# airl-iisc/MRFP

Measured on AMD Instinct MI355X. Metric: train images/sec, higher is better.
Workload: dtype bf16; 1 GPU; resnet-101 DeepLabV3+ + MRFP+ (HRFP+NP+ on, HRFP re-drawn every step), 768x768, 16 images/GPU, fwd+bwd+SGD, synthetic 19-class, random-init weights; global_batch=16, parallelism=dp1

## Files before the change

include/mrfp_hip.h:

```cpp
#ifndef MRFP_HIP_H
#define MRFP_HIP_H

#include <stdint.h>

#ifdef __cplusplus
extern "C" {
#endif

typedef enum { MRFP_F32 = 0, MRFP_BF16 = 1, MRFP_F16 = 2 } mrfp_dtype;

int mrfp_version(void);
const char* mrfp_last_error(void);

int64_t mrfp_stats_nslab(int64_t B, int64_t Ho);

int mrfp_stats_fwd(const void* x, int dtype, int64_t B, int64_t Ho, int64_t Wo, int64_t C,
                   int64_t Hs, int64_t Ws, const int32_t* tabH, const int32_t* tabW,
                   float* ws, void* stream);

int mrfp_stats_bwd(const void* dy, const void* x, const void* y, const float* mean,
                   const float* fA, const float* fS, int per_image, int dtype, int64_t B, int64_t Ho, int64_t Wo, int64_t C,
                   int64_t Hs, int64_t Ws, const int32_t* tabH, const int32_t* tabW,
                   float* ws, void* stream);
int mrfp_stats_bwd_mask(const void* dy, const void* x, const void* mask, const float* mean, int per_image, int dtype, int64_t B,
// ... 22 lines not shown
int mrfp_np_bwd_finalize(const float* ws, int64_t B, int64_t nslab, int64_t count, int64_t C,
                         const float* alpha, const float* beta_noise, const float* mu,
                         const float* sigma, float* Gtmp , float* K, void* stream);

int mrfp_mean_finalize(const float* ws, int64_t B, int64_t nslab, int64_t count, int64_t C,
                       float* tmp, void* out, int dtype, void* stream);

int mrfp_affine_fwd(const void* x, const void* res, void* y, int dtype,
                    int64_t B, int64_t Ho, int64_t Wo, int64_t C, int64_t Hs, int64_t Ws,
                    const int32_t* tabH, const int32_t* tabW,
                    const float* A, const float* S, int coef_per_image, int relu, void* stream);

int mrfp_affine_fwd_stats(const void* x, const void* res, void* y, int dtype, int64_t B, int64_t H, int64_t W, int64_t C,
                          const float* A, const float* S, int coef_per_image, int relu, float* ws, void* stream);
int mrfp_affine_bwd(const void* dy, const void* x, const void* y, void* dx, void* dres, int dtype,
                    int64_t B, int64_t Ho, int64_t Wo, int64_t C, int64_t Hs, int64_t Ws,
                    const int32_t* invH, const int32_t* invW,
                    const float* P, const float* Q, const float* R,
                    const float* fA, const float* fS, int coef_per_image, void* stream);
int mrfp_affine_fwd_relu_mask(const void* x, const void* res, void* y, void* mask, int dtype, int64_t B, int64_t H, int64_t W,
                              int64_t C, const float* A, const float* S, int coef_per_image, void* stream);
int mrfp_affine_bwd_mask(const void* dy, const void* x, const void* mask, void* dx, void* dres, int dtype, int64_t B, int64_t H,
                         int64_t W, int64_t C, const float* P, const float* Q, const float* R, int coef_per_image, void* stream);

int mrfp_copy_channels(const void* src, void* dst, int dtype, int64_t npix, int64_t C, int64_t ld_src, int64_t c0_src,
                       int64_t ld_dst, int64_t c0_dst, void* stream);

int mrfp_add(const void* a, const void* b, void* y, int dtype, int64_t n, void* stream);

int mrfp_bilinear_fwd(const void* x, const void* addend, void* y, int dtype,
                      int64_t B, int64_t Hi, int64_t Wi, int64_t Ho, int64_t Wo, int64_t C, int64_t ld_in,
                      void* stream);
int mrfp_bilinear_bwd(const void* dy, void* dx, int dtype,
                      int64_t B, int64_t Hi, int64_t Wi, int64_t Ho, int64_t Wo, int64_t C, int64_t ld_in,
                      void* stream);
int mrfp_bilinear_fwd_into(const void* x, void* y, int dtype, int64_t B, int64_t Hi, int64_t Wi, int64_t Ho, int64_t Wo,
                           int64_t C, int64_t ld_in, int64_t ld_out, void* stream);
int mrfp_bilinear_bwd_from(const void* dy, void* dx, int dtype, int64_t B, int64_t Hi, int64_t Wi, int64_t Ho, int64_t Wo,
                           int64_t C, int64_t ld_in, int64_t ld_dy, void* stream);

int mrfp_maxpool_fwd(const void* x, void* y, uint8_t* idx, int dtype,
                     int64_t B, int64_t H, int64_t W, int64_t C, void* stream);
int mrfp_maxpool_bwd(const void* dy, const uint8_t* idx, void* dx, int dtype,
                     int64_t B, int64_t H, int64_t W, int64_t C, void* stream);

int mrfp_maxpool_affine_fwd(const void* x, const float* A, const float* S, int coef_per_image, int relu, void* y, uint8_t* idx,
// ... 199 lines not shown
```

mrfp_amd/conv.py:

```python
from __future__ import annotations

import collections
import ctypes
import os as _os
import warnings
import weakref
from typing import Any, NamedTuple, Optional

import torch

from . import _lib
from ._lib import call, dt, ptr, stream
from .ops import CL, GRAD_DEFERRED, _chk, channel_sums, empty_cl, grad_sink, notify_grad, wgrad_workspace, zeros_cl
from .ops import _inside_autograd_engine as _in_backward

_PACKS = {}
FUSE_STATS = [_os.environ.get("MRFP_FUSE_STATS", "1") != "0"]


class ConvStats(NamedTuple):
    final: torch.Tensor
    final_count: int
    elements: int
    rows: torch.Tensor
# ... 653 lines not shown
            side = _WGRADS.stream(x.device) if sink is not None else None
            if sink is not None and GROUP_WGRAD[0] and L_single(B, H, W, Cphys, Ho, Wo, Nphys, x.element_size()):
                _WGRADS.submit(sig, x, dy, sink, weight)
            elif side is not None:
                _WGRADS.ensure_callback()
                _launch_wgrads(sig, [(x, dy, sink)], side)
                notify_grad(weight)
            else:
                dw = sink if sink is not None else torch.empty((N, C, R, S), dtype=torch.float32, device=x.device)
                _launch_wgrads(sig, [(x, dy, dw)], None)
                if sink is not None:
                    notify_grad(weight)
                    dw = None
                elif dw.dtype != weight.dtype:
                    dw = dw.to(weight.dtype)
        if bias is not None and ctx.needs_input_grad[2]:
            db = channel_sums(dy, N).to(bias.dtype)
        return (dx, dw, db) + (None,) * 8


class _SharedConv1x1Pair(torch.autograd.Function):

    @staticmethod
    def forward(ctx, x1, x2, weight, bias, Nphys):
        N, C, R, S = weight.shape
        if R != 1 or S != 1 or x1.shape[1] != C or x2.shape[1] != C:
            raise _lib.MrfpHipError("shared conv pair: 1x1 weight and unpadded inputs expected")
        pk = get_pack(weight, bias, x1.dtype, C, Nphys)
        ys = []
        for x, b in ((x1, None), (x2, pk.bias)):
            B, _, H, W = x.shape
            y = empty_cl(B, Nphys, H, W, x.dtype, x.device)
            call("mrfp_conv_fwd", ptr(x), ptr(pk.wf), ptr(b), ptr(y), dt(x), B, H, W, C, Nphys, Nphys, 1, 1, H, W, 1, 0, 0, 1, 1,
                 None, None, stream())
            ys.append(y)
        ctx.save_for_backward(x1, x2, weight, bias)
        ctx.Nphys = Nphys
        ctx.lr_cell = getattr(x2, "_mrfp_uses", None) if getattr(x2, "_mrfp_lowrank_ok", False) else None
        ctx.set_materialize_grads(False)
        return ys[0], ys[1]

    @staticmethod
    def backward(ctx, dy1, dy2):
        x1, x2, weight, bias = ctx.saved_tensors
        N, C, _, _ = weight.shape
        Nphys = ctx.Nphys
        pk = get_pack(weight, bias, x1.dtype, C, Nphys)
        dxs, dws = [], []
        db = None
        for x, dy, need_dx, cell in ((x1, dy1, ctx.needs_input_grad[0], None), (x2, dy2, ctx.needs_input_grad[1], ctx.lr_cell)):
            if dy is None:
                dxs.append(None)
                continue
            dy = _chk(dy, "dy")
# ... 4 lines not shown
                dx = torch.empty((), dtype=x.dtype, device=x.device).expand(B, C, H, W)
                dx._mrfp_lowrank = (dy, pk.wd, Nphys, dx._version)
                cell[2] = True
            elif need_dx:
                dx = empty_cl(B, C, H, W, x.dtype, x.device)
                call("mrfp_conv_fwd", ptr(dy), ptr(pk.wd), None, ptr(dx), dt(dy), B, H, W, Nphys, C, C, 1, 1, H, W, 1, 0, 0, 1, 1,
                     None, None, stream())
            dxs.append(dx)
            if ctx.needs_input_grad[2]:
                dw = torch.empty((N, C, 1, 1), dtype=torch.float32, device=x.device)
                _launch_wgrads((x.dtype, B, H, W, C, C, N, Nphys, 1, 1, H, W, 1, 0, 0, 1), [(x, dy, dw)], None)
                dws.append(dw)
        if bias is not None and ctx.needs_input_grad[3] and dy2 is not None:
            db = channel_sums(_chk(dy2, "dy"), N).to(bias.dtype)
        dw = None
        if dws:
            total = dws[0] if len(dws) == 1 else dws[0].add_(dws[1])
            sink = grad_sink(weight)
            if sink is not None:
                sink.copy_(total)
                notify_grad(weight)
            else:
                dw = total.to(weight.dtype)
        return dxs[0], dxs[1], dw, db, None


def shared_conv1x1_pair(x1, x2, weight, bias, phys_out):
    return _SharedConv1x1Pair.apply(_chk(x1), _chk(x2), weight, bias, int(phys_out))


def pad_input_channels(x: torch.Tensor, dtype) -> torch.Tensor:
    if not x.is_cuda:
        raise _lib.MrfpHipError("input must live on the GPU (got %s): the HIP path has no CPU fallback" % x.device)
    B, C, H, W = x.shape
    Cpad = _round_up(C, _epc(dtype))
    xs = x.detach()
    if xs.dtype != torch.float32 or not xs.is_contiguous():
        xs = xs.float().contiguous()
    y = empty_cl(B, Cpad, H, W, dtype, x.device)
    call("mrfp_nchw_to_nhwc_pad", ptr(xs), ptr(y), _lib._DT[dtype], B, C, H, W, Cpad, stream())
    return y


def conv2d(x, weight, bias, stride, padding, dilation, phys_out: Optional[int] = None, want_skip: bool = False,
           groups: int = 1, stat_resize=None):
    st = stride[0] if isinstance(stride, (tuple, list)) else int(stride)
    ph, pw = (padding if isinstance(padding, (tuple, list)) else (int(padding), int(padding)))
    dl = dilation[0] if isinstance(dilation, (tuple, list)) else int(dilation)
    N, C = weight.shape[0], weight.shape[1]
    epc = _epc(x.dtype)
    if x.shape[1] % epc != 0:
# ... 46 lines not shown
```

mrfp_amd/csrc/affine.hip:

```cpp
#include "common.hpp"

namespace mrfp {

template <typename T, int VEC, bool RESIZE>
__global__ __launch_bounds__(kThreads) void affine_fwd_kernel(const T* __restrict__ x, const T* __restrict__ res,
                                                              T* __restrict__ y, RowGeom g, int ly,
                                                              const float* __restrict__ A, const float* __restrict__ S,
                                                              int coef_per_image, int relu, uint8_t* __restrict__ mask_out) {
    const int b = blockIdx.x / ly, j = blockIdx.x % ly;
    const Lanes L = make_lanes(g.C, VEC);
    const int t = threadIdx.x;
    const int tcol = t % L.colthreads, trow = t / L.colthreads;
    if (trow >= L.rowthreads) return;
    const size_t cbase = (size_t)(coef_per_image ? b : 0) * g.C;
    for (int cv = tcol; cv < L.lpr; cv += kThreads) {
        float a[VEC], s[VEC];
#pragma unroll
        for (int i = 0; i < VEC; ++i) { a[i] = 1.f; s[i] = 0.f; }
        if (A) load_coef<VEC>(A + cbase + (size_t)cv * VEC, a);
        if (S) load_coef<VEC>(S + cbase + (size_t)cv * VEC, s);
        for (int oh = j; oh < g.Ho; oh += ly) {
            const int ih = RESIZE ? g.tabH[oh] : oh;
            const T* xl = x ? x + ((size_t)b * g.Hs + ih) * g.Ws * g.C + (size_t)cv * VEC : nullptr;
            const size_t dl = ((size_t)b * g.Ho + oh) * g.Wo * g.C + (size_t)cv * VEC;
// ... 107 lines not shown
                            const float vr = inside ? to_f(from_f<T>(v[i])) : 0.f;
                            su[i] += vr;
                            sq[i] += vr * vr;
                        }
                    }
                }
            }
        }
        __syncthreads();
#pragma unroll
        for (int i = 0; i < VEC; ++i) {
            sm[(t * 2 + 0) * VEC + i] = su[i];
            sm[(t * 2 + 1) * VEC + i] = sq[i];
        }
        __syncthreads();
        const int nout = L.colthreads * 2 * VEC;
        for (int o = t; o < nout; o += kThreads) {
            const int oc = o / (2 * VEC), rest = o % (2 * VEC);
            if (cv0 + oc < L.lpr) {
                float acc = 0.f;
                for (int r = 0; r < L.rowthreads; ++r) acc += sm[((r * L.colthreads + oc) * 2) * VEC + rest];
                const int stat = rest / VEC, i = rest % VEC;
                out[(size_t)stat * g.C + (size_t)(cv0 + oc) * VEC + i] = acc;
            }
        }
    }
}

template <typename T, int VEC, int KR, bool YM = false>
__global__ __launch_bounds__(kThreads) void affine_bwd_kernel(const T* __restrict__ dy, const T* __restrict__ x,
                                                              const T* __restrict__ y, T* __restrict__ dx,
                                                              T* __restrict__ dres, RowGeom g, int ly,
                                                              const int32_t* __restrict__ invH,
                                                              const int32_t* __restrict__ invW,
                                                              const float* __restrict__ P, const float* __restrict__ Q,
                                                              const float* __restrict__ R, const float* __restrict__ fA,
                                                              const float* __restrict__ fS, int coef_per_image) {
    const int b = blockIdx.x / ly, j = blockIdx.x % ly;
    const Lanes L = make_lanes(g.C, VEC);
    const int t = threadIdx.x;
    const int tcol = t % L.colthreads, trow = t / L.colthreads;
    if (trow >= L.rowthreads) return;
    const size_t cbase = (size_t)(coef_per_image ? b : 0) * g.C;
    for (int cv = tcol; cv < L.lpr; cv += kThreads) {
        float p[VEC], q[VEC], r[VEC], fa[VEC], fs[VEC];
#pragma unroll
// ... 217 lines not shown
}

template <typename T>
static int launch_affine_fwd(const void* x, const void* res, void* y, int64_t B, int64_t Ho, int64_t Wo, int64_t C,
                             int64_t Hs, int64_t Ws, const int32_t* tabH, const int32_t* tabW, const float* A,
                             const float* S, int cpi, int relu, hipStream_t st, uint8_t* mask_out = nullptr) {
    RowGeom g{(int)B, (int)Ho, (int)Wo, (int)C, (int)Hs, (int)Ws, tabH, tabW};
    const int ly = lines_per_image(B, Ho);
    dim3 grid((unsigned)(B * ly));
    const bool vec_ok = pick_vec<T>(C) > 1 && (!x || aligned16(x)) && aligned16(y) && (!res || aligned16(res)) &&
                        (!A || aligned16(A)) && (!S || aligned16(S));
    if (mask_out && !(vec_ok && FullVec<T>::value == 8)) { set_error("affine_fwd_mask: 16-bit activations with C %% 8 == 0, 16-byte aligned"); return -1; }
    const bool resize = tabH != nullptr || tabW != nullptr;
    if (resize && !(tabH && tabW)) { set_error("affine_fwd: both index tables or none"); return -1; }
    auto launch = [&](auto rs) {
        constexpr bool RS = decltype(rs)::value != 0;
        MRFP_LAUNCH_VEC(vec_ok, (affine_fwd_kernel<T, FullVec<T>::value, RS>), (affine_fwd_kernel<T, 1, RS>), grid, st, (const T*)x,
                        (const T*)res, (T*)y, g, ly, A, S, cpi, relu, mask_out);
        return 0;
    };
    return resize ? launch(Int<1>{}) : launch(Int<0>{});
}

template <typename T>
static int launch_affine_bwd(const void* dy, const void* x, const void* y, void* dx, void* dres, int64_t B, int64_t Ho,
                             int64_t Wo, int64_t C, int64_t Hs, int64_t Ws, const int32_t* invH, const int32_t* invW,
                             const float* P, const float* Q, const float* R, const float* fA, const float* fS, int cpi,
                             hipStream_t st, bool ymask = false) {
    RowGeom g{(int)B, (int)Ho, (int)Wo, (int)C, (int)Hs, (int)Ws, nullptr, nullptr};
    const int ly = lines_per_image(B, Hs);
    dim3 grid((unsigned)(B * ly));
    const bool vec_ok = pick_vec<T>(C) > 1 && aligned16(dy) && aligned16(dx) && (!x || aligned16(x)) &&
                        (!y || aligned16(y)) && (!dres || aligned16(dres)) && (!P || aligned16(P)) &&
                        (!Q || aligned16(Q)) && (!R || aligned16(R)) && (!fA || (aligned16(fA) && aligned16(fS)));
    int kr = 0;
    if (invH && invW && !y && !dres) {
        const int64_t kh = (Ho + Hs - 1) / Hs, kw = (Wo + Ws - 1) / Ws;
        const int64_t k = kh > kw ? kh : kw;
        kr = k <= 3 ? (int)k : 0;
    }
    const bool identity = !invH && !invW;
    if (ymask) {
        if constexpr (FullVec<T>::value == 8) {
            if (!(vec_ok && identity && y)) { set_error("affine_bwd_mask: 16-bit activations, C %% 8 == 0, identity geometry"); return -1; }
            hipLaunchKernelGGL((affine_bwd_kernel<T, 8, -1, true>), grid, dim3(kThreads), 0, st, (const T*)dy, (const T*)x, (const T*)y,
                               (T*)dx, (T*)dres, g, ly, invH, invW, P, Q, R, fA, fS, cpi);
// ... 69 lines not shown
                    const float* P, const float* Q, const float* R, const float* fA, const float* fS, int coef_per_image,
                    void* stream) {
    MRFP_CHECK(!fA == !fS, "affine_bwd: fA and fS go together");
    MRFP_CHECK(dy && dx && B > 0 && Ho > 0 && Wo > 0 && C > 0 && Hs > 0 && Ws > 0, "affine_bwd: bad arguments");
    MRFP_CHECK((invH && invW) || (Hs == Ho && Ws == Wo), "affine_bwd: resize geometry without inverse tables");
    MRFP_CHECK(!dres || (!invH && !invW), "affine_bwd: dres is not supported behind a resize");
    hipStream_t st = (hipStream_t)stream;
    return by_dtype(dtype, "affine_bwd", [&](auto t) {
        using T = typename decltype(t)::type;
        return launch_affine_bwd<T>(dy, x, y, dx, dres, B, Ho, Wo, C, Hs, Ws, invH, invW, P, Q, R, fA, fS, coef_per_image, st);
    });
}

int mrfp_affine_fwd_relu_mask(const void* x, const void* res, void* y, void* mask, int dtype, int64_t B, int64_t H, int64_t W,
                              int64_t C, const float* A, const float* S, int coef_per_image, void* stream) {
    MRFP_CHECK(x && y && mask && A && S && B > 0 && H > 0 && W > 0 && C > 0 && (C & 7) == 0, "affine_fwd_relu_mask: bad arguments");
    hipStream_t st = (hipStream_t)stream;
    return by_dtype16(dtype, "affine_fwd_relu_mask", [&](auto t) {
        using T = typename decltype(t)::type;
        return launch_affine_fwd<T>(x, res, y, B, H, W, C, H, W, nullptr, nullptr, A, S, coef_per_image, 1, st, (uint8_t*)mask);
    });
}

int mrfp_affine_bwd_mask(const void* dy, const void* x, const void* mask, void* dx, void* dres, int dtype, int64_t B, int64_t H,
                         int64_t W, int64_t C, const float* P, const float* Q, const float* R, int coef_per_image, void* stream) {
    MRFP_CHECK(dy && dx && mask && B > 0 && H > 0 && W > 0 && C > 0 && (C & 7) == 0, "affine_bwd_mask: bad arguments");
    hipStream_t st = (hipStream_t)stream;
    return by_dtype16(dtype, "affine_bwd_mask", [&](auto t) {
        using T = typename decltype(t)::type;
        return launch_affine_bwd<T>(dy, x, mask, dx, dres, B, H, W, C, H, W, nullptr, nullptr, P, Q, R, nullptr, nullptr, coef_per_image, st, true);
    });
}

int mrfp_copy_channels(const void* src, void* dst, int dtype, int64_t npix, int64_t C, int64_t ld_src, int64_t c0_src,
                       int64_t ld_dst, int64_t c0_dst, void* stream) {
    MRFP_CHECK(src && dst && npix > 0 && C > 0 && c0_src >= 0 && c0_dst >= 0 && c0_src + C <= ld_src && c0_dst + C <= ld_dst,
               "copy_channels: bad arguments");
    hipStream_t st = (hipStream_t)stream;
    return by_dtype(dtype, "copy_channels", [&](auto t) {
        using T = typename decltype(t)::type;
        return launch_copy_channels<T>(src, dst, npix, C, ld_src, c0_src, ld_dst, c0_dst, st);
    });
}

int mrfp_add(const void* a, const void* b, void* y, int dtype, int64_t n, void* stream) {
    MRFP_CHECK(a && b && y && n > 0, "add: bad arguments");
// ... 9 lines not shown
```

mrfp_amd/deepv3.py:

```python
from __future__ import annotations

import math
import random

import torch
from torch import nn

from . import ops
from .config import cfg
from .conv import wgrad_boundary
from .loss import fused_ce_kwargs, fused_loss
from .network import Resnet
from .network.mynn import (HipBatchNorm2d, HipConv2d, HipInstanceNorm2d, Norm2d, Upsample, conv_norm, initialize_weights,
                           initialize_weights_kaimingnormal_forOC)

__all__ = ["_AtrousSpatialPyramidPoolingModule", "MRFPPlus", "simpleDeepV3Plus", "ReferenceRandom", "InjectedRandom"]


class ReferenceRandom:

    _py = random

    def toggles(self):
        return self._py.random(), self._py.random(), self._py.random()

    def seed_toggles(self, seed):
        self._py = random.Random(seed)

    def reinit_hrfp(self, model):
        flat = _hrfp_arena(model)
        if flat is not None:
            flat[0].normal_()
            flat[0].mul_(flat[1])
        else:
            for conv, bn in model.hrfp_layers():
                initialize_weights_kaimingnormal_forOC(conv)
                initialize_weights_kaimingnormal_forOC(bn)
        from . import conv as conv_mod
        conv_mod.repack_weights([c.weight for c, _ in model.hrfp_layers()], tag="hrfp",
# ... 175 lines not shown
        if isinstance(trunk, Resnet.ResNet3X3):
            return trunk.stem(x, w_arr), w_arr
        return Resnet._conv_norm_relu_pool(self.layer0[0], self.layer0[1], trunk.wt_layer[2], ops.as_activation(x), w_arr), w_arr

    def _low(self, t, w_arr):
        if hasattr(self, "layer1"):
            return self.layer1([wgrad_boundary(t), w_arr])[0]
        return self.mod3(wgrad_boundary(t))

    def _high(self, t, w_arr, fourier=None):
        if hasattr(self, "layer1"):
            t = self.layer2([wgrad_boundary(t), w_arr])
            if fourier is not None:
                t[0] = fourier.at("layer2", t[0])
            self._tap("layer2", t[0])
            t[0] = wgrad_boundary(t[0])
            t = self.layer3(t)
            self._tap("layer3", t[0])
            t[0] = wgrad_boundary(t[0])
            return wgrad_boundary(self.layer4(t)[0])
        t = self.mod7(self.mod6(self.mod5(wgrad_boundary(self.mod4(wgrad_boundary(t))))))
        return wgrad_boundary(self.bn_out[0].fused(t, relu=True))

    def _final1(self, d):
        d = conv_norm(self.final1[0], self.final1[1], d, relu=True)
        return conv_norm(self.final1[3], self.final1[4], d, relu=True)

    def _head(self, dec1, size, gts, training, low_res=False):
        f2 = self.final2[0]
        nc = f2.out_channels
        pitch = (nc + 31) // 32 * 32
        dec2 = ops.conv2d(dec1, f2.weight, f2.bias, f2.stride, f2.padding, f2.dilation, phys_out=pitch)
        if low_res:
            if training:
                raise ValueError("low_res is an eval-path option (training=False)")
            return dec2
        if training and cfg.MODEL.FUSE_UPSAMPLE_CE and fused_ce_kwargs(self.criterion) is not None:
            return fused_loss(self.criterion, dec2, gts, size, nc)
        main_out = ops.upsample_bilinear(dec2, size, channels=nc)
        if training:
            return self._loss(main_out, gts)
        return main_out.float()

    def _head_o2(self, dec1, oc_dec, size, gts, training):
        from . import conv
        f2 = self.final2[0]
        nc = f2.out_channels
        pitch = (nc + 31) // 32 * 32
        p_low, p_half = conv.shared_conv1x1_pair(dec1, oc_dec, f2.weight, f2.bias, pitch)
        dec2 = ops.upsample_bilinear(p_low, (oc_dec.shape[2], oc_dec.shape[3]), addend=p_half)
        if training and cfg.MODEL.FUSE_UPSAMPLE_CE and fused_ce_kwargs(self.criterion) is not None:
            return fused_loss(self.criterion, dec2, gts, size, nc)
        main_out = ops.upsample_bilinear(dec2, size, channels=nc)
        if training:
            return self._loss(main_out, gts)
        return main_out.float()

    def _loss(self, main_out, gts):
        loss = fused_loss(self.criterion, main_out, gts)
        if loss is None:
            loss = self.criterion(main_out.float(), gts)
        return loss


class MRFPPlus(_DeepLabBase):
    _allow_101 = True

    def __init__(self, num_classes, trunk="resnet-50", criterion=None, criterion_aux=None,
                 variant="D16", wt_layer=[0, 0, 4, 4, 4, 0, 0], use_wtloss=False):
        super().__init__()
        self.criterion = criterion
        self.criterion_aux = criterion_aux
# ... 12 lines not shown
        for i, (ci, co, d) in enumerate(dec, 1):
            setattr(self, "OCdeclayer%d" % i, HipConv2d(ci, co, kernel_size=3, stride=1, padding=d, dilation=d).requires_grad_(False))
            setattr(self, "OC%d_decbn" % i, HipBatchNorm2d(co).requires_grad_(False))
        for conv, bn in self.hrfp_layers():
            initialize_weights_kaimingnormal_forOC(conv)
            initialize_weights_kaimingnormal_forOC(bn)
        self._init_head()
        self.rng = ReferenceRandom()
        self.fourier_perturb = None

    def _fold_skips_hrfp(self):
        return (getattr(self, "_mrfp_fold", False) and not self.training and not torch.is_grad_enabled())

    def hrfp_layers(self):
        enc = [(getattr(self, "OClayer%d" % i), getattr(self, "OC%d_bn" % i)) for i in range(1, 5)]
        dec = [(getattr(self, "OCdeclayer%d" % i), getattr(self, "OC%d_decbn" % i)) for i in range(1, 5)]
        return enc + dec

    def Normalization_Perturbation_Plus(self, feat, which="np1", res=None):
        B, C = feat.shape[0], feat.shape[1]
        alpha, beta_noise = self.rng.np_noise(which, B, C, feat.device)
        return ops.np_plus(feat, alpha, beta_noise, res)

    def _hrfp(self, xp, h, w, need_out=True, need_dec=True):
        lazy = (cfg.MODEL.HRFP_LAZY or self._fold_skips_hrfp()) and self._taps is None
        if lazy and not (need_out or need_dec):
            return None, None, xp
        resize = [dict(scale=1.205), dict(scale=1.2), dict(scale=1.2), dict(size=(int(h / 2), int(w / 2))),
                  dict(size=(int(h / 2), int(w / 2))), dict(scale=0.838), dict(scale=0.798),
                  dict(size=(math.ceil(h / 4), math.ceil(w / 4)))]
        t, dec, xp_alias = xp, None, xp
        for i, ((conv, bn), rs) in enumerate(zip(self.hrfp_layers(), resize)):
            if i == 4 and lazy and not need_out:
                return t, None, xp_alias
            plan = ops.nearest_plan(t.shape[2], t.shape[3], device=t.device, **rs)
            stat_resize = plan if bn.training else None
            if i == 0:
                t, xp_alias = conv.forward_skip(t, stat_resize=stat_resize)
            elif i == 4:
                t, dec = conv.forward_skip(t, stat_resize=stat_resize)
            else:
                t = conv(t, stat_resize=stat_resize)
            if (plan.Hs, plan.Ws) != tuple(t.shape[2:]):
                plan = ops.nearest_plan(t.shape[2], t.shape[3], device=t.device, **rs)
            t = bn.fused(t, relu=True, plan=plan)
            self._tap("hrfp%d" % i, t)
        return dec, t, xp_alias

    def forward(self, x, gts=None, training=True, low_res=False):
        if low_res and training:
            raise ValueError("low_res is an eval-path option (training=False)")
        p, p2, p3 = self.rng.toggles()
        h, w = x.shape[2], x.shape[3]
        o1, npp, o2 = (training == True and p < 0.5), (training == True and p2 < 0.5), (training == True and p3 < 0.5)
        if o1:
            self.rng.reinit_hrfp(self)

        xp, w_arr = self._stem(x)
        fourier = None
        if training == True and self.fourier_perturb is not None:
            fp = self.fourier_perturb
            if hasattr(fp, "begin"):
                fp.begin(x.shape[0], True)
                xp = fp.at("stem", xp)
                fourier = fp
            else:
                xp = fp(xp)
        self._tap("stem", xp)
        OCout_dec, OCout, xp = self._hrfp(xp, h, w, o1, o2)
        t = xp
        if npp and o1 and self._taps is None:
            t = self.Normalization_Perturbation_Plus(xp, "np1", res=OCout)
        else:
            if npp:
                t = self.Normalization_Perturbation_Plus(xp, "np1")
                self._tap("np1", t)
            if o1:
                t = ops.add(OCout, t)
        tap = getattr(self.layer1[-1], "instance_norm_layer", None) if hasattr(self, "layer1") else None
        if isinstance(tap, HipInstanceNorm2d):
            tap._emit_plane_stats = bool(npp) and fourier is None
        t = self._low(t, w_arr)
        if fourier is not None:
            t = fourier.at("layer1", t)
        if npp:
            t = self.Normalization_Perturbation_Plus(t, "np2")
        self._tap("layer1", t)
        dec0_fine, low_level = self.bot_fine.forward_skip(t)
        t = self._high(low_level, w_arr, fourier)
        if self.use_wtloss:
            self.w_arr = w_arr
        self._tap("layer4", t)
        t = self.aspp(t)
        self._tap("aspp", t)
        dec0_up = self.bot_aspp(t)
        dec1 = self._final1(ops.concat_upsample(dec0_fine, dec0_up, low_level.shape[2:], cfg.MODEL.DECODER_PAD))
        self._tap("dec1", dec1)
        if o2:
            if cfg.MODEL.COMMUTE_O2:
                return self._head_o2(dec1, OCout_dec, (h, w), gts, training)
            dec1 = ops.upsample_bilinear(dec1, (int(h / 2), int(w / 2)), addend=OCout_dec)
        return self._head(dec1, (h, w), gts, training, low_res)


class simpleDeepV3Plus(_DeepLabBase):
    _allow_101 = False

    def __init__(self, num_classes, trunk="resnet-50", criterion=None, criterion_aux=None,
                 variant="D16", wt_layer=[0, 0, 0, 0, 0, 0, 0], use_wtloss=False):
        super().__init__()
        self.criterion = criterion
        self.criterion_aux = criterion_aux
        self.variant = variant
        self.wt_layer = wt_layer
        self.use_wtloss = use_wtloss
        self.trunk = trunk
        self._build_trunk_and_head(num_classes, trunk, wt_layer)
        self._init_head()

    def forward(self, x, gts=None, training=False, low_res=False):
        h, w = x.shape[2], x.shape[3]
        t, w_arr = self._stem(x)
        x_tuple = self.layer1([t, w_arr])
# ... 7 lines not shown
```

mrfp_amd/network/mynn.py:

```python
from __future__ import annotations

import torch
import torch.nn as nn

from .. import ops
from ..config import cfg


class HipBatchNorm2d(nn.BatchNorm2d):

    _nbt_pending = 0

    def _flush_nbt(self):
        if self._nbt_pending and self.num_batches_tracked is not None:
            self.num_batches_tracked.add_(self._nbt_pending)
        self._nbt_pending = 0

    def _save_to_state_dict(self, destination, prefix, keep_vars):
        self._flush_nbt()
        super()._save_to_state_dict(destination, prefix, keep_vars)

    def _load_from_state_dict(self, *args, **kwargs):
        self._nbt_pending = 0
        super()._load_from_state_dict(*args, **kwargs)

    def fused(self, x, *, relu=False, res=None, plan=None, emit_stats=False):
        training = self.training or (self.running_mean is None)
        if training and self.num_batches_tracked is not None:
            self._nbt_pending += 1
        return ops.batch_norm_act(x, self.weight, self.bias,
                                  self.running_mean if self.track_running_stats else None,
                                  self.running_var if self.track_running_stats else None,
                                  training=training, momentum=self.momentum, eps=self.eps,
                                  relu=relu, res=res, plan=plan, emit_stats=emit_stats)

    def forward(self, x):
        return self.fused(x)


class HipInstanceNorm2d(nn.InstanceNorm2d):

    _emit_plane_stats = False

    def fused(self, x, *, relu=False):
        return ops.instance_norm_act(x, self.weight, self.bias, eps=self.eps, relu=relu, emit_stats=self._emit_plane_stats)

    def fused_relu_pool(self, x):
        return ops.instance_norm_relu_pool(x, self.weight, self.bias, eps=self.eps)

    def forward(self, x):
        return self.fused(x)


class HipLocalBatchNorm2d(HipBatchNorm2d):

    def fused(self, x, *, act=None):
        training = self.training or (self.running_mean is None)
# ... 115 lines not shown
```

mrfp_amd/ops.py:

```python
from __future__ import annotations

import collections
import math
import os
import weakref
from functools import lru_cache
from typing import Optional, Tuple

import numpy as np
import torch

from . import _lib
from ._lib import call, dt, ptr, stream

CL = torch.channels_last

GRAD_NOTIFY = [None]
GRAD_DEFERRED = set()


def wgrad_workspace(M, N, Q, device, n=1):
    return torch.empty(int(_lib.lib().mrfp_conv_wgrad_grouped_ws_bytes(M, N, Q, n)), dtype=torch.uint8, device=device)


# ... 266 lines not shown
        if total is None:
            total = _SYNC_BN_COUNTS[key] = int(round(tot[2 * C].item()))
        else:
            flag = _SYNC_BN_FLAG.get(ws.device)
            if flag is None:
                flag = _SYNC_BN_FLAG[ws.device] = torch.zeros(1, dtype=torch.int32, device=ws.device)
            flag.add_((tot[2 * C:2 * C + 1] != float(total)).to(torch.int32))
    return torch.stack([hi, lo]).contiguous(), total


ACT_NONE, ACT_RELU, ACT_RELU6 = 0, 1, 2
GATED_BN_HITS = [0]
GATED_BN = [os.environ.get("MRFP_GATED_BN", "1") != "0"]
RELU6_GATE_HITS = [0]


def _keeps_sign_mask(x, relu, res, plan):
    return bool(relu and res is not None and plan is None and SIGN_MASK[0] and x.element_size() == 2 and x.shape[1] % 8 == 0)


class _BatchNormAct(torch.autograd.Function):

    @staticmethod
    def forward(ctx, x, weight, bias, running_mean, running_var, res, training, momentum, eps, act, plan, may_sync, stats):
        relu, relu6 = act == ACT_RELU, act == ACT_RELU6
        if relu6 and (res is not None or plan is not None):
            raise _lib.MrfpHipError("BatchNorm + ReLU6 takes no residual and no resize plan")
        x = _chk(x)
        res = _chk(res, "res") if res is not None else None
        B, Ho, Wo, C, Hs, Ws, *_ = _geom(x, plan)
        dev = x.device
        w32, b32 = _f32(weight), _f32(bias)
        coef = torch.empty(4 * C, dtype=torch.float32, device=dev)
        mean, invstd, A, S = coef[0:C], coef[C:2 * C], coef[2 * C:3 * C], coef[3 * C:4 * C]
        if training:
            fused = _serving_colstats(x, C, B * Ho * Wo, plan, False)
            if fused is not None:
                ws, nb_, nslab = fused.final, 1, fused.final_count
            else:
                nslab, ws = _stats_fwd(x, plan)
                nb_ = B
            count = B * Ho * Wo
            ctx.sync = _sync_bn_group() if may_sync else None
            if ctx.sync is not None:
                ws, count = _allreduce_stats(ws, nb_ * nslab, C, count, ctx.sync)
                nb_, nslab = 1, 2
            ctx.count = count
            call("mrfp_bn_finalize", ptr(ws), nb_, nslab, count, C, ptr(w32), ptr(b32), float(eps),
                 float(momentum), ptr(running_mean), ptr(running_var), ptr(mean), ptr(invstd), ptr(A), ptr(S), stream())
        else:
            ctx.sync, ctx.count = None, B * Ho * Wo
            call("mrfp_bn_eval_coef", C, ptr(w32), ptr(b32), ptr(running_mean), ptr(running_var), float(eps),
                 ptr(A), ptr(S), stream())
            if x.requires_grad or (weight is not None and weight.requires_grad):
                mean.copy_(running_mean)
                torch.rsqrt(running_var.float() + eps, out=invstd)
        ctx.plan, ctx.act, ctx.training, ctx.has_res = plan, act, training, res is not None
        ctx.keep_y = relu and res is not None
        ctx.remask = relu and res is None
        ctx.ymask = _keeps_sign_mask(x, relu, res, plan)
        ctx.gate_skip = bool(ctx.ymask and GATED_SKIP[0] and getattr(res, "_mrfp_skip_alias", False))
        ctx.gate_ok = bool(act == ACT_NONE and res is None and plan is None and training and x.element_size() == 2 and C % 8 == 0)
        ctx.alias_uses = getattr(res, "_mrfp_uses", None)
        keep = None
        if relu6:
            y = empty_cl(B, C, Ho, Wo, x.dtype, dev)
            keep = torch.empty((B * Ho * Wo * C + 7) // 8, dtype=torch.uint8, device=dev)
            call("mrfp_affine_fwd_relu6_mask", ptr(x), ptr(y), ptr(keep), dt(x), B * Ho * Wo, C, ptr(A), ptr(S), stream())
        elif ctx.ymask:
            y = empty_cl(B, C, Ho, Wo, x.dtype, dev)
            keep = torch.empty(B * Ho * Wo * C // 8, dtype=torch.uint8, device=dev)
            call("mrfp_affine_fwd_relu_mask", ptr(x), ptr(res), ptr(y), ptr(keep), dt(x), B, Ho, Wo, C, ptr(A), ptr(S), 0, stream())
        else:
            y = _affine_fwd(x, res, A, S, False, relu, plan, stats=stats)
            if ctx.keep_y:
                keep = y
        ctx.wparam, ctx.bparam = weight, bias
        ctx.save_for_backward(x, keep, w32, mean, invstd, A, S)
        return y

    @staticmethod
    def backward(ctx, dy):
        x, keep, w32, mean, invstd, A, S = ctx.saved_tensors
        gate = None
        cell = getattr(ctx, "_mrfp_cell", None)
        g = getattr(dy, "_mrfp_gate", None)
        if cell is not None and cell[1]:
            if g is None or g[1] != dy._version:
                raise _lib.MrfpHipError("a gated gradient reached its BatchNorm without its gate: the layer's output was also "
                                        "consumed by an operator outside mrfp_amd.ops (set MRFP_GATED_SKIP=0)")
            cell[1] = False
        if g is not None:
            if (g[1] == dy._version and ctx.gate_ok and dy.dtype == x.dtype and dy.shape == x.shape
                    and dy.is_contiguous(memory_format=CL)):
                gate = g[0]
            else:
                from .conv import ungate
                dy = ungate(dy)
        dy = _chk(dy, "dy")
        plan = ctx.plan
        B, Ho, Wo, C, *_ = _geom(x, plan)
        fA, fS = (A, S) if ctx.remask else (None, None)
        mask = y = None
        if gate is not None:
            mask = gate
            GATED_BN_HITS[0] += 1
# ... 21 lines not shown
        call("mrfp_bn_bwd_finalize", ptr(ws), B, nslab, B * Ho * Wo, C, ptr(w32), ptr(mean), ptr(invstd),
             ptr(dw), ptr(db), ptr(P), ptr(Q), ptr(R), stream())
        if ctx.sync is not None:
            gws, _ = _allreduce_stats(ws, B * nslab, C, 0, ctx.sync)
            call("mrfp_bn_bwd_finalize", ptr(gws), 1, 2, ctx.count, C, ptr(w32), ptr(mean), ptr(invstd), None, None,
                 ptr(P), ptr(Q), ptr(R), stream())
        if not ctx.training:
            Q.zero_()
            R.zero_()
        if mask is not None:
            dx = empty_cl(B, C, Ho, Wo, dy.dtype, dy.device)
            dres = dres_out = None
            if ctx.ymask:
                if ctx.gate_skip and ctx.needs_input_grad[5] and ctx.alias_uses is not None and ctx.alias_uses[0] == 1:
                    dres = dy.view_as(dy)
                    dres._mrfp_gate = (mask, dres._version)
                    ctx.alias_uses[1] = True
                else:
                    dres = dres_out = empty_cl(B, C, Ho, Wo, dy.dtype, dy.device)
            call("mrfp_affine_bwd_mask", ptr(dy), ptr(x), ptr(mask), ptr(dx), ptr(dres_out), dt(dy), B, Ho, Wo, C, ptr(P), ptr(Q),
                 ptr(R), 0, stream())
        else:
            dx, dres = _affine_bwd(dy, x, y, P, Q, R, False, plan, ctx.has_res, x, fA, fS)
        return (dx, _grad_result(ctx.wparam, dw), _grad_result(ctx.bparam, db), None, None, dres) + (None,) * 7


RUNNING_STATS_EPOCH = [0]


def batch_norm_act(x, weight, bias, running_mean, running_var, *, training, momentum=0.1, eps=1e-5,
                   relu=False, res=None, plan=None, emit_stats=False):
    if training and running_mean is not None:
        RUNNING_STATS_EPOCH[0] += 1
    ps = _planestats_rows(x, emit_stats and plan is None and not _keeps_sign_mask(x, relu, res, plan))
    y = _BatchNormAct.apply(x, weight, bias, running_mean, running_var, res, training, momentum, eps,
                            ACT_RELU if relu else ACT_NONE, plan, True, ps[1] if ps is not None else None)
    _tag_planestats(y, ps)
    if (GATED_BN[0] and GATED_SKIP[0] and SIGN_MASK[0] and not relu and res is None and plan is None and training and y.grad_fn is not None
            and y.element_size() == 2 and y.shape[1] % 8 == 0):
        y._mrfp_skip_alias = True
        y._mrfp_uses = [0, False]
        y.grad_fn._mrfp_cell = y._mrfp_uses
    return y


def local_batch_norm_act(x, weight, bias, running_mean, running_var, *, training, momentum=0.1, eps=1e-5, act=None):
    if act not in (None, "relu6"):
        raise _lib.MrfpHipError("local_batch_norm_act: act must be None or 'relu6' (got %r)" % (act,))
    if training and running_mean is not None:
        RUNNING_STATS_EPOCH[0] += 1
    return _BatchNormAct.apply(x, weight, bias, running_mean, running_var, None, bool(training), momentum, eps,
                               ACT_RELU6 if act == "relu6" else ACT_NONE, None, False, None)


def batch_norm_relu6(x, weight, bias, running_mean, running_var, *, training, momentum=0.1, eps=1e-5):
    return local_batch_norm_act(x, weight, bias, running_mean, running_var, training=training, momentum=momentum, eps=eps,
                                act="relu6")


IN_FUSED_STATS = [os.environ.get("MRFP_IN_FUSED_STATS", "1") != "0"]
IN_FUSED_HITS = [0]


def _in_plane_sums(x):
    ps = _take_planestats(x)
    x = _chk(x)
# ... 1356 lines not shown
```

Measured before the change: 309.3 images/sec.

## Fuse final 1x1 classifier conv into BatchNorm-ReLU epilogue for both head branches

Adds a kernel that applies the BN affine/ReLU (with optional nearest resize) and, in the same pass, runs the 1x1 final2 classifier conv with MFMA on the freshly written tile, emitting class scores alongside the activation. The HRFP stage-3 BN and the final1 BN now produce p_half and p_low directly, so the shared 1x1 conv pair skips its forward launches and the re-read of the two large feature maps. The cost is extra LDS use and register pressure in the BN kernel. The forward path is also restricted to bf16/f16, C<=256 and N<=32 shapes, with the old path kept as a fallback.

New measurement: 310.8 images/sec, median of 6. About the same (+0.5%).

```diff
diff --git a/include/mrfp_hip.h b/include/mrfp_hip.h
--- a/include/mrfp_hip.h
+++ b/include/mrfp_hip.h
@@ -68,6 +68,11 @@
                               int64_t C, const float* A, const float* S, int coef_per_image, void* stream);
 int mrfp_affine_bwd_mask(const void* dy, const void* x, const void* mask, void* dx, void* dres, int dtype, int64_t B, int64_t H,
                          int64_t W, int64_t C, const float* P, const float* Q, const float* R, int coef_per_image, void* stream);
+int mrfp_affine_fwd_scores(const void* x, const void* res, void* y, void* mask, int dtype, int64_t B, int64_t Ho, int64_t Wo, int64_t C,
+                           int64_t Hs, int64_t Ws, const int32_t* tabH, const int32_t* tabW, const float* A, const float* S,
+                           int coef_per_image, int relu, const void* wpack, const float* bias, int64_t N, void* scores, int64_t ldp,
+                           void* stream);
+int mrfp_affine_scores_ok(int dtype, int64_t C, int64_t N, int64_t ldp);
 
 int mrfp_copy_channels(const void* src, void* dst, int dtype, int64_t npix, int64_t C, int64_t ld_src, int64_t c0_src,
                        int64_t ld_dst, int64_t c0_dst, void* stream);
diff --git a/mrfp_amd/conv.py b/mrfp_amd/conv.py
--- a/mrfp_amd/conv.py
+++ b/mrfp_amd/conv.py
@@ -699,14 +699,19 @@
 class _SharedConv1x1Pair(torch.autograd.Function):
 
     @staticmethod
-    def forward(ctx, x1, x2, weight, bias, Nphys):
+    def forward(ctx, x1, x2, weight, bias, Nphys, y1=None, y2=None):
         N, C, R, S = weight.shape
         if R != 1 or S != 1 or x1.shape[1] != C or x2.shape[1] != C:
             raise _lib.MrfpHipError("shared conv pair: 1x1 weight and unpadded inputs expected")
         pk = get_pack(weight, bias, x1.dtype, C, Nphys)
         ys = []
-        for x, b in ((x1, None), (x2, pk.bias)):
+        for x, b, pre in ((x1, None, y1), (x2, pk.bias, y2)):
             B, _, H, W = x.shape
+            if pre is not None:
+                if pre.shape != (B, Nphys, H, W) or pre.dtype != x.dtype or not pre.is_contiguous(memory_format=CL):
+                    raise _lib.MrfpHipError("shared conv pair: a precomputed output must be the launch's [B,%d,H,W] channels-last tensor" % Nphys)
+                ys.append(pre.detach())
+                continue
             y = empty_cl(B, Nphys, H, W, x.dtype, x.device)
             call("mrfp_conv_fwd", ptr(x), ptr(pk.wf), ptr(b), ptr(y), dt(x), B, H, W, C, Nphys, Nphys, 1, 1, H, W, 1, 0, 0, 1, 1,
                  None, None, stream())
@@ -757,11 +762,11 @@
                 notify_grad(weight)
             else:
                 dw = total.to(weight.dtype)
-        return dxs[0], dxs[1], dw, db, None
-
-
-def shared_conv1x1_pair(x1, x2, weight, bias, phys_out):
-    return _SharedConv1x1Pair.apply(_chk(x1), _chk(x2), weight, bias, int(phys_out))
+        return dxs[0], dxs[1], dw, db, None, None, None
+
+
+def shared_conv1x1_pair(x1, x2, weight, bias, phys_out, y1=None, y2=None):
+    return _SharedConv1x1Pair.apply(_chk(x1), _chk(x2), weight, bias, int(phys_out), y1, y2)
 
 
 def pad_input_channels(x: torch.Tensor, dtype) -> torch.Tensor:
diff --git a/mrfp_amd/csrc/affine.hip b/mrfp_amd/csrc/affine.hip
--- a/mrfp_amd/csrc/affine.hip
+++ b/mrfp_amd/csrc/affine.hip
@@ -1,4 +1,4 @@
-#include "common.hpp"
+#include "conv_common.hpp"
 
 namespace mrfp {
 
@@ -153,6 +153,109 @@
                 for (int r = 0; r < L.rowthreads; ++r) acc += sm[((r * L.colthreads + oc) * 2) * VEC + rest];
                 const int stat = rest / VEC, i = rest % VEC;
                 out[(size_t)stat * g.C + (size_t)(cv0 + oc) * VEC + i] = acc;
+            }
+        }
+    }
+}
+
+template <typename T, bool RESIZE, int KS>
+__global__ __launch_bounds__(kThreads) void affine_fwd_scores_kernel(const T* __restrict__ x, const T* __restrict__ res,
+                                                                     T* __restrict__ y, RowGeom g, int ly,
+                                                                     const float* __restrict__ A, const float* __restrict__ S,
+                                                                     int coef_per_image, int relu, uint8_t* __restrict__ mask_out,
+                                                                     const T* __restrict__ wpack, const float* __restrict__ bias, int N,
+                                                                     T* __restrict__ scores) {
+    constexpr int VEC = 8, CT = 4 * KS, RT = kThreads / CT, PT = 4 * RT, NB = (PT + 15) / 16, PITCH = (CT + 1) * 16;
+    extern __shared__ __attribute__((aligned(16))) char tile[];
+    const int b = blockIdx.x / ly, j = blockIdx.x % ly;
+    const int t = threadIdx.x, lane = t & 63, l15 = lane & 15, lq = lane >> 4;
+    const int wave = __builtin_amdgcn_readfirstlane(t >> 6);
+    const int tcol = t % CT, trow = t / CT;
+    const bool active = trow < RT;
+    const size_t cbase = (size_t)(coef_per_image ? b : 0) * g.C;
+    const int jj = wave & 1;
+    uint4 fw[KS];
+#pragma unroll
+    for (int ks = 0; ks < KS; ++ks) {
+        const int n = 8 * (l15 >> 2) + 4 * jj + (l15 & 3);
+        fw[ks] = n < N ? *reinterpret_cast<const uint4*>(wpack + (size_t)n * g.C + ks * 32 + lq * 8) : make_uint4(0u, 0u, 0u, 0u);
+    }
+    const int nl = 8 * lq + 4 * jj;
+    float bv[4];
+#pragma unroll
+    for (int e = 0; e < 4; ++e) bv[e] = (bias && nl + e < N) ? bias[nl + e] : 0.f;
+    float a[VEC], s[VEC];
+#pragma unroll
+    for (int i = 0; i < VEC; ++i) { a[i] = 1.f; s[i] = 0.f; }
+    if (active) {
+        if (A) load_coef<VEC>(A + cbase + (size_t)tcol * VEC, a);
+        if (S) load_coef<VEC>(S + cbase + (size_t)tcol * VEC, s);
+    }
+    for (int oh = j; oh < g.Ho; oh += ly) {
+        const int ih = RESIZE ? g.tabH[oh] : oh;
+        const T* xl = x + ((size_t)b * g.Hs + ih) * g.Ws * g.C + (size_t)tcol * VEC;
+        const size_t dl = ((size_t)b * g.Ho + oh) * g.Wo * g.C + (size_t)tcol * VEC;
+        for (int owb = 0; owb < g.Wo; owb += PT) {
+            VecT<T, VEC> xr[4], rr[4];
+            int owc[4], iwv[4];
+            if (active) {
+#pragma unroll
+                for (int u = 0; u < 4; ++u) {
+                    owc[u] = min(owb + trow + u * RT, g.Wo - 1);
+                    iwv[u] = RESIZE ? g.tabW[owc[u]] : owc[u];
+                }
+#pragma unroll
+                for (int u = 0; u < 4; ++u) {
+                    xr[u] = RESIZE ? load_raw<T, VEC>(xl + (size_t)iwv[u] * g.C) : load_raw_nt<T, VEC>(xl + (size_t)iwv[u] * g.C);
+                    if (res) rr[u] = load_raw_nt<T, VEC>(res + dl + (size_t)owc[u] * g.C);
+                }
+            }
+            __syncthreads();
+            if (active) {
+#pragma unroll
+                for (int u = 0; u < 4; ++u) {
+                    const int ow = owb + trow + u * RT;
+                    if (ow >= g.Wo) continue;
+                    float v[VEC];
+                    cvt_f<T, VEC>(xr[u], v);
+#pragma unroll
+                    for (int i = 0; i < VEC; ++i) v[i] = v[i] * a[i] + s[i];
+                    if (res) {
+                        float r[VEC];
+                        cvt_f<T, VEC>(rr[u], r);
+#pragma unroll
+                        for (int i = 0; i < VEC; ++i) v[i] += r[i];
+                    }
+                    if (relu) {
+#pragma unroll
+                        for (int i = 0; i < VEC; ++i) v[i] = v[i] > 0.f ? v[i] : 0.f;
+                    }
+                    VecT<T, VEC> tv;
+#pragma unroll
+                    for (int i = 0; i < VEC; ++i) tv.v[i] = from_f<T>(v[i]);
+                    *reinterpret_cast<VecT<T, VEC>*>(y + dl + (size_t)ow * g.C) = tv;
+                    *reinterpret_cast<VecT<T, VEC>*>(tile + (trow + u * RT) * PITCH + tcol * 16) = tv;
+                    if (mask_out) {
+                        unsigned m = 0;
+#pragma unroll
+                        for (int i = 0; i < VEC; ++i) m |= (to_f(tv.v[i]) > 0.f ? 1u : 0u) << i;
+                        mask_out[(dl + (size_t)ow * g.C) >> 3] = (uint8_t)m;
+                    }
+                }
+            }
+            __syncthreads();
+            for (int pb = wave >> 1; pb < NB && owb + pb * 16 < g.Wo; pb += 2) {
+                f32x4 acc = {0.f, 0.f, 0.f, 0.f};
+                const char* frag = tile + (pb * 16 + l15) * PITCH + lq * 16;
+#pragma unroll
+                for (int ks = 0; ks < KS; ++ks) Mma16<T>::run(acc, fw[ks], *reinterpret_cast<const uint4*>(frag + ks * 64));
+                const int ow = owb + pb * 16 + l15;
+                if (ow < g.Wo) {
+                    VecT<T, 4> o;
+#pragma unroll
+                    for (int e = 0; e < 4; ++e) o.v[e] = from_f<T>(acc[e] + bv[e]);
+                    *reinterpret_cast<VecT<T, 4>*>(scores + (((size_t)b * g.Ho + oh) * g.Wo + ow) * 32 + nl) = o;
+                }
             }
         }
     }
@@ -416,6 +519,41 @@
     return resize ? launch(Int<1>{}) : launch(Int<0>{});
 }
 
+static bool affine_scores_shape_ok(int64_t C, int64_t N, int64_t ldp) { return C > 0 && C <= 256 && C % 32 == 0 && N > 0 && N <= 32 && ldp == 32; }
+
+template <typename T>
+static int launch_affine_fwd_scores(const void* x, const void* res, void* y, uint8_t* mask_out, int64_t B, int64_t Ho, int64_t Wo,
+                                    int64_t C, int64_t Hs, int64_t Ws, const int32_t* tabH, const int32_t* tabW, const float* A,
+                                    const float* S, int cpi, int relu, const void* wpack, const float* bias, int64_t N, void* scores,
+                                    hipStream_t st) {
+    RowGeom g{(int)B, (int)Ho, (int)Wo, (int)C, (int)Hs, (int)Ws, tabH, tabW};
+    const int ly = lines_per_image(B, Ho);
+    dim3 grid((unsigned)(B * ly));
+    const bool resize = tabH != nullptr || tabW != nullptr;
+    auto launch = [&](auto rs, auto ks) {
+        constexpr bool RS = decltype(rs)::value != 0;
+        constexpr int KS = decltype(ks)::value;
+        constexpr int CT = 4 * KS, PT = 4 * (kThreads / CT), NB = (PT + 15) / 16;
+        hipLaunchKernelGGL((affine_fwd_scores_kernel<T, RS, KS>), grid, dim3(kThreads), (size_t)(NB * 16 * (CT + 1) * 16), st, (const T*)x,
+                           (const T*)res, (T*)y, g, ly, A, S, cpi, relu, mask_out, (const T*)wpack, bias, (int)N, (T*)scores);
+        MRFP_LAUNCH_CHECK();
+        return 0;
+    };
+    auto by_ks = [&](auto rs) {
+        switch ((int)(C / 32)) {
+        case 1: return launch(rs, Int<1>{});
+        case 2: return launch(rs, Int<2>{});
+        case 3: return launch(rs, Int<3>{});
+        case 4: return launch(rs, Int<4>{});
+        case 5: return launch(rs, Int<5>{});
+        case 6: return launch(rs, Int<6>{});
+        case 7: return launch(rs, Int<7>{});
+        default: return launch(rs, Int<8>{});
+        }
+    };
+    return resize ? by_ks(Int<1>{}) : by_ks(Int<0>{});
+}
+
 template <typename T>
 static int launch_affine_bwd(const void* dy, const void* x, const void* y, void* dx, void* dres, int64_t B, int64_t Ho,
                              int64_t Wo, int64_t C, int64_t Hs, int64_t Ws, const int32_t* invH, const int32_t* invW,
@@ -531,6 +669,28 @@
     });
 }
 
+int mrfp_affine_scores_ok(int dtype, int64_t C, int64_t N, int64_t ldp) {
+    return ((dtype == MRFP_BF16 || dtype == MRFP_F16) && affine_scores_shape_ok(C, N, ldp)) ? 1 : 0;
+}
+
+int mrfp_affine_fwd_scores(const void* x, const void* res, void* y, void* mask, int dtype, int64_t B, int64_t Ho, int64_t Wo, int64_t C,
+                           int64_t Hs, int64_t Ws, const int32_t* tabH, const int32_t* tabW, const float* A, const float* S,
+                           int coef_per_image, int relu, const void* wpack, const float* bias, int64_t N, void* scores, int64_t ldp,
+                           void* stream) {
+    MRFP_CHECK(x && y && wpack && scores && B > 0 && Ho > 0 && Wo > 0 && C > 0 && Hs > 0 && Ws > 0, "affine_fwd_scores: bad arguments");
+    MRFP_CHECK((tabH && tabW) || (!tabH && !tabW && Hs == Ho && Ws == Wo), "affine_fwd_scores: resize geometry without both index tables");
+    hipStream_t st = (hipStream_t)stream;
+    return by_dtype16(dtype, "affine_fwd_scores", [&](auto t) {
+        using T = typename decltype(t)::type;
+        MRFP_CHECK(affine_scores_shape_ok(C, N, ldp), "affine_fwd_scores: C %% 32 == 0, C <= 256, N <= 32 and ldp == 32 (see mrfp_affine_scores_ok)");
+        MRFP_CHECK(aligned16(x) && aligned16(y) && aligned16(wpack) && aligned16(scores) && (!res || aligned16(res)) &&
+                       (!A || aligned16(A)) && (!S || aligned16(S)),
+                   "affine_fwd_scores: tensors, coefficients and the weight pack must be 16-byte aligned");
+        return launch_affine_fwd_scores<T>(x, res, y, (uint8_t*)mask, B, Ho, Wo, C, Hs, Ws, tabH, tabW, A, S, coef_per_image, relu, wpack,
+                                           bias, N, scores, st);
+    });
+}
+
 int mrfp_affine_bwd_mask(const void* dy, const void* x, const void* mask, void* dx, void* dres, int dtype, int64_t B, int64_t H,
                          int64_t W, int64_t C, const float* P, const float* Q, const float* R, int coef_per_image, void* stream) {
     MRFP_CHECK(dy && dx && mask && B > 0 && H > 0 && W > 0 && C > 0 && (C & 7) == 0, "affine_bwd_mask: bad arguments");
diff --git a/mrfp_amd/deepv3.py b/mrfp_amd/deepv3.py
--- a/mrfp_amd/deepv3.py
+++ b/mrfp_amd/deepv3.py
@@ -15,6 +15,8 @@
                            initialize_weights_kaimingnormal_forOC)
 
 __all__ = ["_AtrousSpatialPyramidPoolingModule", "MRFPPlus", "simpleDeepV3Plus", "ReferenceRandom", "InjectedRandom"]
+
+HEAD_SCORES = [__import__("os").environ.get("MRFP_HEAD_SCORES", "1") != "0"]
 
 
 class ReferenceRandom:
@@ -236,8 +238,10 @@
         t = self.mod7(self.mod6(self.mod5(wgrad_boundary(self.mod4(wgrad_boundary(t))))))
         return wgrad_boundary(self.bn_out[0].fused(t, relu=True))
 
-    def _final1(self, d):
+    def _final1(self, d, head=None):
         d = conv_norm(self.final1[0], self.final1[1], d, relu=True)
+        if head is not None:
+            return self.final1[4].fused_scores(self.final1[3](d), head[:1] + (None,) + head[2:], relu=True)
         return conv_norm(self.final1[3], self.final1[4], d, relu=True)
 
     def _head(self, dec1, size, gts, training, low_res=False):
@@ -256,12 +260,12 @@
             return self._loss(main_out, gts)
         return main_out.float()
 
-    def _head_o2(self, dec1, oc_dec, size, gts, training):
+    def _head_o2(self, dec1, oc_dec, size, gts, training, p_low=None, p_half=None):
         from . import conv
         f2 = self.final2[0]
         nc = f2.out_channels
         pitch = (nc + 31) // 32 * 32
-        p_low, p_half = conv.shared_conv1x1_pair(dec1, oc_dec, f2.weight, f2.bias, pitch)
+        p_low, p_half = conv.shared_conv1x1_pair(dec1, oc_dec, f2.weight, f2.bias, pitch, p_low, p_half)
         dec2 = ops.upsample_bilinear(p_low, (oc_dec.shape[2], oc_dec.shape[3]), addend=p_half)
         if training and cfg.MODEL.FUSE_UPSAMPLE_CE and fused_ce_kwargs(self.criterion) is not None:
             return fused_loss(self.criterion, dec2, gts, size, nc)
@@ -320,17 +324,30 @@
         alpha, beta_noise = self.rng.np_noise(which, B, C, feat.device)
         return ops.np_plus(feat, alpha, beta_noise, res)
 
-    def _hrfp(self, xp, h, w, need_out=True, need_dec=True):
+    def _score_head(self, dtype, training):
+        from . import conv
+        f2 = self.final2[0]
+        C, pitch = f2.in_channels, (f2.out_channels + 31) // 32 * 32
+        norms = (self.OC4_bn, self.final1[4])
+        if not (HEAD_SCORES[0] and training == True and cfg.MODEL.COMMUTE_O2 and self._taps is None and hasattr(self, "layer1")
+                and all(type(n) is HipBatchNorm2d and n.num_features == C for n in norms)
+                and tuple(f2.kernel_size) == (1, 1) and ops.affine_scores_ok(dtype, C, pitch, pitch)):
+            return None
+        pk = conv.get_pack(f2.weight, f2.bias, dtype, C, pitch)
+        return (pk.wf, pk.bias, pitch, pitch)
+
+    def _hrfp(self, xp, h, w, need_out=True, need_dec=True, head=None):
+        p_half = None
         lazy = (cfg.MODEL.HRFP_LAZY or self._fold_skips_hrfp()) and self._taps is None
         if lazy and not (need_out or need_dec):
-            return None, None, xp
+            return None, None, xp, None
         resize = [dict(scale=1.205), dict(scale=1.2), dict(scale=1.2), dict(size=(int(h / 2), int(w / 2))),
                   dict(size=(int(h / 2), int(w / 2))), dict(scale=0.838), dict(scale=0.798),
                   dict(size=(math.ceil(h / 4), math.ceil(w / 4)))]
         t, dec, xp_alias = xp, None, xp
         for i, ((conv, bn), rs) in enumerate(zip(self.hrfp_layers(), resize)):
             if i == 4 and lazy and not need_out:
-                return t, None, xp_alias
+                return t, None, xp_alias, p_half
             plan = ops.nearest_plan(t.shape[2], t.shape[3], device=t.device, **rs)
             stat_resize = plan if bn.training else None
             if i == 0:
@@ -341,9 +358,12 @@
                 t = conv(t, stat_resize=stat_resize)
             if (plan.Hs, plan.Ws) != tuple(t.shape[2:]):
                 plan = ops.nearest_plan(t.shape[2], t.shape[3], device=t.device, **rs)
-            t = bn.fused(t, relu=True, plan=plan)
+            if i == 3 and head is not None:
+                t, p_half = bn.fused_scores(t, head, relu=True, plan=plan)
+            else:
+                t = bn.fused(t, relu=True, plan=plan)
             self._tap("hrfp%d" % i, t)
-        return dec, t, xp_alias
+        return dec, t, xp_alias, p_half
 
     def forward(self, x, gts=None, training=True, low_res=False):
         if low_res and training:
@@ -365,7 +385,8 @@
             else:
                 xp = fp(xp)
         self._tap("stem", xp)
-        OCout_dec, OCout, xp = self._hrfp(xp, h, w, o1, o2)
+        head = self._score_head(xp.dtype, training) if o2 else None
+        OCout_dec, OCout, xp, p_half = self._hrfp(xp, h, w, o1, o2, head)
         t = xp
         if npp and o1 and self._taps is None:
             t = self.Normalization_Perturbation_Plus(xp, "np1", res=OCout)
@@ -392,11 +413,14 @@
         t = self.aspp(t)
         self._tap("aspp", t)
         dec0_up = self.bot_aspp(t)
-        dec1 = self._final1(ops.concat_upsample(dec0_fine, dec0_up, low_level.shape[2:], cfg.MODEL.DECODER_PAD))
+        dec1 = self._final1(ops.concat_upsample(dec0_fine, dec0_up, low_level.shape[2:], cfg.MODEL.DECODER_PAD), head)
+        p_low = None
+        if head is not None:
+            dec1, p_low = dec1
         self._tap("dec1", dec1)
         if o2:
             if cfg.MODEL.COMMUTE_O2:
-                return self._head_o2(dec1, OCout_dec, (h, w), gts, training)
+                return self._head_o2(dec1, OCout_dec, (h, w), gts, training, p_low, p_half)
             dec1 = ops.upsample_bilinear(dec1, (int(h / 2), int(w / 2)), addend=OCout_dec)
         return self._head(dec1, (h, w), gts, training, low_res)
 
diff --git a/mrfp_amd/network/mynn.py b/mrfp_amd/network/mynn.py
--- a/mrfp_amd/network/mynn.py
+++ b/mrfp_amd/network/mynn.py
@@ -33,6 +33,15 @@
                                   self.running_var if self.track_running_stats else None,
                                   training=training, momentum=self.momentum, eps=self.eps,
                                   relu=relu, res=res, plan=plan, emit_stats=emit_stats)
+
+    def fused_scores(self, x, head, *, relu=False, plan=None):
+        training = self.training or (self.running_mean is None)
+        if training and self.num_batches_tracked is not None:
+            self._nbt_pending += 1
+        return ops.batch_norm_act_scores(x, self.weight, self.bias,
+                                         self.running_mean if self.track_running_stats else None,
+                                         self.running_var if self.track_running_stats else None, head,
+                                         training=training, momentum=self.momentum, eps=self.eps, relu=relu, plan=plan)
 
     def forward(self, x):
         return self.fused(x)
diff --git a/mrfp_amd/ops.py b/mrfp_amd/ops.py
--- a/mrfp_amd/ops.py
+++ b/mrfp_amd/ops.py
@@ -312,7 +312,7 @@
 class _BatchNormAct(torch.autograd.Function):
 
     @staticmethod
-    def forward(ctx, x, weight, bias, running_mean, running_var, res, training, momentum, eps, act, plan, may_sync, stats):
+    def forward(ctx, x, weight, bias, running_mean, running_var, res, training, momentum, eps, act, plan, may_sync, stats, head=None):
         relu, relu6 = act == ACT_RELU, act == ACT_RELU6
         if relu6 and (res is not None or plan is not None):
             raise _lib.MrfpHipError("BatchNorm + ReLU6 takes no residual and no resize plan")
@@ -353,7 +353,21 @@
         ctx.gate_ok = bool(act == ACT_NONE and res is None and plan is None and training and x.element_size() == 2 and C % 8 == 0)
         ctx.alias_uses = getattr(res, "_mrfp_uses", None)
         keep = None
-        if relu6:
+        scores = None
+        if head is not None:
+            if relu6 or stats is not None:
+                raise _lib.MrfpHipError("BatchNorm with class scores takes no ReLU6 and emits no plane statistics")
+            wpack, hbias, hN, ldp = head
+            _, _, _, _, _, _, tH, tW, _, _ = _geom(x, plan)
+            y = empty_cl(B, C, Ho, Wo, x.dtype, dev)
+            scores = empty_cl(B, ldp, Ho, Wo, x.dtype, dev)
+            if ctx.ymask:
+                keep = torch.empty(B * Ho * Wo * C // 8, dtype=torch.uint8, device=dev)
+            call("mrfp_affine_fwd_scores", ptr(x), ptr(res), ptr(y), ptr(keep), dt(x), B, Ho, Wo, C, Hs, Ws, ptr(tH), ptr(tW), ptr(A),
+                 ptr(S), 0, int(relu), ptr(wpack), ptr(hbias), hN, ptr(scores), ldp, stream())
+            if keep is None and ctx.keep_y:
+                keep = y
+        elif relu6:
             y = empty_cl(B, C, Ho, Wo, x.dtype, dev)
             keep = torch.empty((B * Ho * Wo * C + 7) // 8, dtype=torch.uint8, device=dev)
             call("mrfp_affine_fwd_relu6_mask", ptr(x), ptr(y), ptr(keep), dt(x), B * Ho * Wo, C, ptr(A), ptr(S), stream())
@@ -367,11 +381,18 @@
                 keep = y
         ctx.wparam, ctx.bparam = weight, bias
         ctx.save_for_backward(x, keep, w32, mean, invstd, A, S)
+        if scores is not None:
+            ctx.mark_non_differentiable(scores)
+            ctx.set_materialize_grads(False)
+            return y, scores
         return y
 
     @staticmethod
-    def backward(ctx, dy):
+    def backward(ctx, dy, _dscores=None):
         x, keep, w32, mean, invstd, A, S = ctx.saved_tensors
+        if dy is None:
+            Bz, Hz, Wz, Cz, *_ = _geom(x, ctx.plan)
+            dy = zeros_cl(Bz, Cz, Hz, Wz, x.dtype, x.device)
         gate = None
         cell = getattr(ctx, "_mrfp_cell", None)
         g = getattr(dy, "_mrfp_gate", None)
@@ -439,7 +460,7 @@
                  ptr(R), 0, stream())
         else:
             dx, dres = _affine_bwd(dy, x, y, P, Q, R, False, plan, ctx.has_res, x, fA, fS)
-        return (dx, _grad_result(ctx.wparam, dw), _grad_result(ctx.bparam, db), None, None, dres) + (None,) * 7
+        return (dx, _grad_result(ctx.wparam, dw), _grad_result(ctx.bparam, db), None, None, dres) + (None,) * 8
 
 
 RUNNING_STATS_EPOCH = [0]
@@ -459,6 +480,18 @@
         y._mrfp_uses = [0, False]
         y.grad_fn._mrfp_cell = y._mrfp_uses
     return y
+
+
+def affine_scores_ok(dtype, C, N, ldp):
+    return dtype in _lib._DT and bool(_lib.lib().mrfp_affine_scores_ok(_lib._DT[dtype], C, N, ldp))
+
+
+def batch_norm_act_scores(x, weight, bias, running_mean, running_var, head, *, training, momentum=0.1, eps=1e-5, relu=False,
+                          plan=None):
+    if training and running_mean is not None:
+        RUNNING_STATS_EPOCH[0] += 1
+    return _BatchNormAct.apply(x, weight, bias, running_mean, running_var, None, training, momentum, eps,
+                               ACT_RELU if relu else ACT_NONE, plan, True, None, head)
 
 
 def local_batch_norm_act(x, weight, bias, running_mean, running_var, *, training, momentum=0.1, eps=1e-5, act=None):
```
